# LouisNUST/pose-unsupervised

Hardware: AMD Instinct MI355X
Metric: 4-view 256x256 frames/sec (fwd+triangulate) (higher is better)
Workload: dtype bf16

## Files before the change

pose-unsupervised_amd/csrc/bottleneck.hip:

```cpp
#include "gemm_common.h"

namespace posu {
namespace {

struct BottleGeom {
  const void* x;
  void* y;
  const void* w1;
  const float* s1;
  const float* b1;
  const void* w2;
  const float* s2;
  const float* b2;
  const void* w3;
  const float* s3;
  const float* b3;
  int N, H;
  int strips;
  int rows;
};

#ifndef POSU_BNECK_ABLATE
#define POSU_BNECK_ABLATE 0
#endif
constexpr int kAbl = POSU_BNECK_ABLATE;


constexpr int kP = 64, kW = 64, kC = 256;
constexpr int kW2 = 0;
constexpr int kW3 = 73728;
constexpr int kT1 = 106496;
constexpr int kSlot = 66 * 128;
constexpr int kBN = kT1 + 3 * kSlot;
constexpr int kXP = kBN + 3072;
constexpr int kXT = kXP + 16384;
constexpr int kLds = kXT + 8192;
static_assert(kLds <= 160 * 1024, "LDS");

__device__ __forceinline__ void raw_barrier() {
  if (kAbl & 8) return;
  lds_barrier();
}

__device__ __forceinline__ void ld8(const float* p, float* v) {
  const float4 a = *reinterpret_cast<const float4*>(p);
  const float4 b = *reinterpret_cast<const float4*>(p + 4);
  v[0] = a.x; v[1] = a.y; v[2] = a.z; v[3] = a.w;
  v[4] = b.x; v[5] = b.y; v[6] = b.z; v[7] = b.w;
}

template <typename T, bool DOWN>
__global__ __launch_bounds__(512, 1) void bottleneck64_kernel(BottleGeom g) {
  using O = Op<T>;
  constexpr int ES = static_cast<int>(sizeof(T));
  static_assert(ES == 2, "bf16 / f16 activations");
  constexpr int kCi = DOWN ? 64 : kC;
  constexpr int NF = DOWN ? 2 : 4;
  constexpr int kW3K = DOWN ? 2 * kP : kP;
  __shared__ __attribute__((aligned(16))) char smem[kLds];

  const int tid = threadIdx.x;
  const int lane = tid & 63, wid = tid >> 6;
  const int r16 = lane & 15, q = lane >> 4;
  const int pg = wid & 3, h = wid >> 2;
  const unsigned lds0 = static_cast<unsigned>(reinterpret_cast<size_t>((__attribute__((address_space(3))) char*)smem));
  const unsigned wid_u = __builtin_amdgcn_readfirstlane(static_cast<unsigned>(wid));

  const int n = blockIdx.x / g.strips;
  const int ya = (blockIdx.x - n * g.strips) * g.rows, yb = ya + g.rows;
  const int H = g.H;
  const int px = 16 * pg + r16;
  const int cq = 16 * (q & 1) + 8 * (q >> 1);
  const float* bn = reinterpret_cast<const float*>(smem + kBN);
  float* xp_mine = reinterpret_cast<float*>(smem + kXP + (2 * pg + h) * 2048 + lane * 32);
  const float* xp_part = reinterpret_cast<const float*>(smem + kXP + (2 * pg + 1 - h) * 2048 + lane * 32);
  uint4* xt_mine = reinterpret_cast<uint4*>(smem + kXT + (2 * pg + h) * 1024 + lane * 16);
  const uint4* xt_part = reinterpret_cast<const uint4*>(smem + kXT + (2 * pg + 1 - h) * 1024 + lane * 16);

  {
    const u32x4 w2s = make_srd(g.w2, kP * 9 * kP * ES);
    const u32x4 w3s = make_srd(g.w3, kC * kW3K * ES);
    const int cL = (tid & 7) ^ ((tid >> 4) & 7), drow = tid >> 3;
#pragma unroll
    for (int t = 0; t < 9; ++t)
      dma16(w2s, (drow * (9 * kP) + t * kP + cL * 8) * ES, lds0 + kW2 + t * 8192 + wid_u * 1024);
#pragma unroll
    for (int i = 0; i < 4; ++i)
      dma16(w3s, ((drow + 64 * i) * kW3K + cL * 8) * ES, lds0 + kW3 + i * 8192 + wid_u * 1024);
    float* bw = reinterpret_cast<float*>(smem + kBN);
    if (tid < 64) {
      bw[tid] = g.s1[tid];
      bw[64 + tid] = g.b1[tid];
      bw[128 + tid] = g.s2[tid];
      bw[192 + tid] = g.b2[tid];
    }
    if (tid < 256) {
      bw[256 + tid] = DOWN ? 1.f : g.s3[tid];
      bw[512 + tid] = g.b3[tid];
    }
    if (tid < 48) {
      const int sl = tid >> 4, side = (tid >> 3) & 1, ch = tid & 7;
      *reinterpret_cast<uint4*>(smem + kT1 + sl * kSlot + side * 65 * 128 + ch * 16) = make_uint4(0, 0, 0, 0);
    }
  }
  uint4 w1f[4][4];
  {
    const T* w1 = reinterpret_cast<const T*>(g.w1);
#pragma unroll
    for (int s = 0; s < 4; ++s)
#pragma unroll
      for (int j = 0; j < 4; ++j) {
        if constexpr (DOWN) {
          if (s < 2 && j < 2) w1f[s][j] = *reinterpret_cast<const uint4*>(w1 + (16 * (2 * h + j) + r16) * kCi + 32 * s + 8 * q);
        } else {
          w1f[s][j] = *reinterpret_cast<const uint4*>(w1 + (16 * ((j + 2 * h) & 3) + r16) * kC + 32 * (4 * h + s) + 8 * q);
        }
      }
  }
  uint4 wdf[2][2][4];
  if constexpr (DOWN) {
    const T* w3 = reinterpret_cast<const T*>(g.w3);
#pragma unroll
    for (int qh = 0; qh < 2; ++qh)
#pragma unroll
      for (int s = 0; s < 2; ++s)
#pragma unroll
        for (int j = 0; j < 4; ++j)
          wdf[qh][s][j] = *reinterpret_cast<const uint4*>(w3 + (128 * h + 64 * qh + 16 * j + r16) * kW3K + kP + 32 * s + 8 * q);
  }

  const __amdgpu_buffer_rsrc_t xrs =
      __builtin_amdgcn_make_buffer_rsrc(const_cast<void*>(g.x), 0, g.N * H * kW * kCi * ES, 0x00020000);
  const __amdgpu_buffer_rsrc_t yrs = __builtin_amdgcn_make_buffer_rsrc(g.y, 0, g.N * H * kW * kC * ES, 0x00020000);
  const int lane_off = (px * kC + 128 * h + cq) * ES;
  const int lane_offx = DOWN ? (px * kCi + 8 * q) * ES : lane_off;
  constexpr int kRowBytes = kW * kC * ES, kRowBytesX = kW * kCi * ES;
  const int rmax = (yb < H - 1 ? yb : H - 1);
  auto load_row = [&](int r, uint4(&f)[4]) {
    const int rr = r < 0 ? 0 : (r > rmax ? rmax : r);
    const int roff = __builtin_amdgcn_readfirstlane((n * H + rr) * kRowBytesX);
    if (kAbl & 32) {
#pragma unroll
      for (int s = 0; s < NF; ++s) f[s] = make_uint4(rr, s, lane, 1);
      return;
    }
#pragma unroll
    for (int s = 0; s < NF; ++s) {
      const auto v = __builtin_amdgcn_raw_buffer_load_b128(xrs, lane_offx + 64 * s, roff, (kAbl & 128) ? 2 : 0);
      f[s] = make_uint4(v[0], v[1], v[2], v[3]);
    }
  };
  auto conv1_part = [&](int r, const uint4(&f)[4], f32x4(&acc)[2]) {
    f32x4 a[4];
#pragma unroll
    for (int j = 0; j < 4; ++j) a[j] = f32x4{0.f, 0.f, 0.f, 0.f};
    if constexpr (DOWN) {
      if (r >= 0 && r < H) {
#pragma unroll
        for (int s = 0; s < 2; ++s)
#pragma unroll
          for (int j = 0; j < 2; ++j) O::mma(a[j], w1f[s][j], f[s]);
      }
      acc[0] = a[0];
      acc[1] = a[1];
      return;
    }
    if (r >= 0 && r < H) {
#pragma unroll
      for (int s = 0; s < 4; ++s)
#pragma unroll
        for (int j = 0; j < 4; ++j) {
          if (kAbl & 16) a[j][0] += __uint_as_float(f[s].x ^ w1f[s][j].y);
          else O::mma(a[j], w1f[s][j], f[s]);
        }
    }
    *reinterpret_cast<f32x4*>(xp_mine) = a[2];
    *reinterpret_cast<f32x4*>(xp_mine + 4) = a[3];
    acc[0] = a[0];
    acc[1] = a[1];
  };
  auto conv1_fin = [&](int r, const f32x4(&acc)[2]) {
    char* slot = smem + kT1 + ((r + 3) % 3) * kSlot;
    const bool ok = r >= 0 && r < H;
    f32x4 t0 = acc[0], t1 = acc[1];
    if constexpr (!DOWN) {
      const f32x4 pa = *reinterpret_cast<const f32x4*>(xp_part);
      const f32x4 pb = *reinterpret_cast<const f32x4*>(xp_part + 4);
#pragma unroll
      for (int e = 0; e < 4; ++e) {
        t0[e] += pa[e];
        t1[e] += pb[e];
      }
    }
    const int c0 = 16 * (2 * h + (q & 1)) + 8 * (q >> 1);
    float v[8], sc[8], sh[8];
#pragma unroll
    for (int e = 0; e < 4; ++e) {
      const auto sw = __builtin_amdgcn_permlane16_swap(__float_as_uint(t0[e]), __float_as_uint(t1[e]), false, false);
      v[e] = __uint_as_float(sw[0]);
      v[4 + e] = __uint_as_float(sw[1]);
    }
    ld8(bn + c0, sc);
    ld8(bn + 64 + c0, sh);
    affine8<!DOWN>(v, sc, sh);
#pragma unroll
    for (int e = 0; e < 8; ++e) v[e] = ok ? fmaxf(v[e], 0.f) : 0.f;
    *reinterpret_cast<uint4*>(slot + swz(px + 1, c0 >> 3)) = O::store_vals(v);
  };
  auto conv2_row = [&](int y, auto&& mid) -> uint4 {
    f32x4 acc2[2];
#pragma unroll
    for (int j = 0; j < 2; ++j) acc2[j] = f32x4{0.f, 0.f, 0.f, 0.f};
#pragma unroll
    for (int t = 0; t < 9; ++t) {
      if (t == 5) mid();
      const int dy = t / 3, dx = t % 3;
      const char* slot = smem + kT1 + ((y - 1 + dy + 3) % 3) * kSlot;
      const char* Wt = smem + kW2 + t * 8192;
#pragma unroll
      for (int cb = 0; cb < 2; ++cb) {
        uint4 wf[2];
#pragma unroll
        for (int j = 0; j < 2; ++j) wf[j] = *reinterpret_cast<const uint4*>(Wt + swz(16 * (2 * h + j) + r16, 4 * cb + q));
        const uint4 tf = *reinterpret_cast<const uint4*>(slot + swz(px + dx, 4 * cb + q));
#pragma unroll
        for (int j = 0; j < 2; ++j) {
          if (kAbl & 1) acc2[j][0] += __uint_as_float(wf[j].x ^ tf.y);
          else O::mma(acc2[j], wf[j], tf);
        }
      }
    }
    const int ca = 32 * h + 4 * q, cb2 = ca + 16;
    const float4 sa = *reinterpret_cast<const float4*>(bn + 128 + ca);
    const float4 sb = *reinterpret_cast<const float4*>(bn + 128 + cb2);
    const float4 ha = *reinterpret_cast<const float4*>(bn + 192 + ca);
    const float4 hb = *reinterpret_cast<const float4*>(bn + 192 + cb2);
    const float s8[8] = {sa.x, sa.y, sa.z, sa.w, sb.x, sb.y, sb.z, sb.w};
    const float h8[8] = {ha.x, ha.y, ha.z, ha.w, hb.x, hb.y, hb.z, hb.w};
    float v[8] = {acc2[0][0], acc2[0][1], acc2[0][2], acc2[0][3], acc2[1][0], acc2[1][1], acc2[1][2], acc2[1][3]};
    affine8<!DOWN>(v, s8, h8);
#pragma unroll
    for (int e = 0; e < 8; ++e) v[e] = fmaxf(v[e], 0.f);
    return O::store_vals(v);
  };
  uint4 pend[4];
  int pend_off = 0;
  auto flush = [&](int k) {
    const uint4 u = pend[k];
    if (kAbl & 4) {
      asm volatile("" ::"v"(u.x), "v"(u.y), "v"(u.z), "v"(u.w));
      return;
    }
    __builtin_amdgcn_raw_buffer_store_b128((__attribute__((ext_vector_type(4))) unsigned){u.x, u.y, u.z, u.w}, yrs,
                                           lane_off + 64 * k + pend_off, 0, (kAbl & 64) ? 2 : 0);
  };
  auto conv3_row = [&](int y, const uint4(&tb)[2], const uint4(&res)[4]) {
    pend_off = __builtin_amdgcn_readfirstlane((n * H + y) * kRowBytes);
#pragma unroll
    for (int qh = 0; qh < 2; ++qh) {
      const int qd = 2 * h + qh;
      f32x4 acc3[4];
#pragma unroll
      for (int j = 0; j < 4; ++j) acc3[j] = f32x4{0.f, 0.f, 0.f, 0.f};
#pragma unroll
      for (int kb = 0; kb < 2; ++kb) {
#pragma unroll
        for (int j = 0; j < 4; ++j) {
          const uint4 wf = *reinterpret_cast<const uint4*>(smem + kW3 + swz(64 * qd + 16 * j + r16, 4 * kb + q));
          if (kAbl & 2) acc3[j][0] += __uint_as_float(wf.x ^ tb[kb].y);
          else O::mma(acc3[j], wf, tb[kb]);
        }
      }
      if constexpr (DOWN) {
#pragma unroll
        for (int s = 0; s < 2; ++s)
#pragma unroll
          for (int j = 0; j < 4; ++j) O::mma(acc3[j], wdf[qh][s][j], res[s]);
      }
#pragma unroll
      for (int jp = 0; jp < 2; ++jp) {
        const int s = 2 * qd + jp, c0 = 32 * s + cq;
        float v[8], r[8], sc[8], sh[8];
#pragma unroll
        for (int e = 0; e < 4; ++e) {
          const auto sw = __builtin_amdgcn_permlane16_swap(__float_as_uint(acc3[2 * jp][e]),
                                                           __float_as_uint(acc3[2 * jp + 1][e]), false, false);
          v[e] = __uint_as_float(sw[0]);
          v[4 + e] = __uint_as_float(sw[1]);
        }
        ld8(bn + 512 + c0, sh);
        if constexpr (DOWN) {
#pragma unroll
          for (int e = 0; e < 8; ++e) v[e] = fmaxf(v[e] + sh[e], 0.f);
        } else {
          ld8(bn + 256 + c0, sc);
          O::load_vals(res[2 * qh + jp], r);
          affine8<!DOWN>(v, sc, sh);
          add8<!DOWN>(v, r);
#pragma unroll
          for (int e = 0; e < 8; ++e) v[e] = fmaxf(v[e], 0.f);
        }
        uint4& pk = pend[2 * qh + jp];
        pk = O::store_vals(v);
        asm("" : "+v"(pk.x), "+v"(pk.y), "+v"(pk.z), "+v"(pk.w));
      }
    }
  };

  uint4 xa[4], xb[4], xc[4], xd[4];
  f32x4 c1[2];
  load_row(ya - 1, xd);
  load_row(ya, xa);
  vm_wait<0>();
  raw_barrier();
  load_row(ya + 1, xb);
  load_row(ya + 2, xc);
  conv1_part(ya - 1, xd, c1);
  if (!DOWN) raw_barrier();
  conv1_fin(ya - 1, c1);
  if (!DOWN) raw_barrier();
  conv1_part(ya, xa, c1);
  if (!DOWN) raw_barrier();
  conv1_fin(ya, c1);

  auto step = [&](int y, const uint4(&ra)[4], const uint4(&rb)[4], uint4(&rd)[4], bool fl) {
    conv1_part(y + 1, rb, c1);
    load_row(y + 3, rd);
    if (fl) flush(0);
    if (!DOWN) raw_barrier();
    conv1_fin(y + 1, c1);
    if (fl) flush(1);
    raw_barrier();
    const uint4 mine = conv2_row(y, [&] { if (fl) flush(2); });
    if (fl) flush(3);
    *xt_mine = mine;
    raw_barrier();
    const uint4 part = *xt_part;
    const uint4 tb[2] = {h ? part : mine, h ? mine : part};
    conv3_row(y, tb, ra);
  };
  step(ya, xa, xb, xd, false);
  int y = ya + 1;
  for (; y + 4 <= yb; y += 4) {
    step(y, xb, xc, xa, true);
    step(y + 1, xc, xd, xb, true);
    step(y + 2, xd, xa, xc, true);
    step(y + 3, xa, xb, xd, true);
  }
  if (y < yb) {
    step(y, xb, xc, xa, true);
    if (y + 1 < yb) step(y + 1, xc, xd, xb, true);
    if (y + 2 < yb) step(y + 2, xd, xa, xc, true);
  }
#pragma unroll
  for (int k = 0; k < 4; ++k) flush(k);
}

}
}

using namespace posu;

namespace {
int bottleneck_launch(bool down, int dtype, const void* x, int N, int H, int W, int C, int P, const void* w1,
                      const float* s1, const float* b1, const void* w2, const float* s2, const float* b2,
                      const void* w3, const float* s3, const float* b3, void* y, void* stream, const char* what) {
  const std::string wh(what);
  POSU_REQUIRE(dtype == POSU_BF16 || dtype == POSU_F16, wh + ": dtype must be BF16 or F16");
  POSU_REQUIRE(x && w1 && s1 && b1 && w2 && s2 && b2 && w3 && (s3 || down) && b3 && y, wh + ": null pointer");
  POSU_REQUIRE(x != y, wh + ": the output must not alias the input");
  POSU_REQUIRE(W == kW && C == (down ? 64 : kC) && P == kP,
               wh + (down ? ": built for W = 64, C = 64, planes = 64 (layer1 block 0 of PoseResNet at 256x256)"
                          : ": built for W = 64, C = 256, planes = 64 (layer1 of PoseResNet at 256x256)"));
  POSU_REQUIRE(N > 0 && H > 0, wh + ": empty input");
  POSU_REQUIRE(static_cast<long long>(N) * H * W * kC * 2 < (1LL << 31) - 256,
               wh + ": activation exceeds the 2 GiB addressing range");
  for (const void* p : {x, static_cast<const void*>(y), w1, w2, w3})
    POSU_REQUIRE((reinterpret_cast<size_t>(p) & 15) == 0, wh + ": pointers must be 16-byte aligned");
  BottleGeom g{};
  g.x = x;
  g.y = y;
  g.w1 = w1;
  g.s1 = s1;
  g.b1 = b1;
  g.w2 = w2;
  g.s2 = s2;
  g.b2 = b2;
  g.w3 = w3;
  g.s3 = s3;
  g.b3 = b3;
  g.N = N;
  g.H = H;
  int strips = 1;
  while (N * strips * 2 <= 256 && H % (strips * 2) == 0 && H / (strips * 2) >= 2) strips *= 2;
  g.strips = strips;
  g.rows = H / strips;
  hipStream_t s = as_stream(stream);
  const dim3 grid(N * strips), block(512);
  if (dtype == POSU_BF16) {
    if (down) hipLaunchKernelGGL((bottleneck64_kernel<uint16_t, true>), grid, block, 0, s, g);
    else hipLaunchKernelGGL((bottleneck64_kernel<uint16_t, false>), grid, block, 0, s, g);
  } else {
    if (down) hipLaunchKernelGGL((bottleneck64_kernel<f16_t, true>), grid, block, 0, s, g);
    else hipLaunchKernelGGL((bottleneck64_kernel<f16_t, false>), grid, block, 0, s, g);
  }
  return check_launch(what);
}
}

extern "C" int posu_bottleneck_fwd(int dtype, const void* x, int N, int H, int W, int C, int P, const void* w1,
                                   const float* s1, const float* b1, const void* w2, const float* s2, const float* b2,
                                   const void* w3, const float* s3, const float* b3, void* y, void* stream) {
  return bottleneck_launch(false, dtype, x, N, H, W, C, P, w1, s1, b1, w2, s2, b2, w3, s3, b3, y, stream,
                           "posu_bottleneck_fwd");
}

extern "C" int posu_bottleneck_down_fwd(int dtype, const void* x, int N, int H, int W, int C, int P,
                                        const void* w1, const float* s1, const float* b1, const void* w2,
                                        const float* s2, const float* b2, const void* w3d, const float* shift3,
                                        void* y, void* stream) {
  return bottleneck_launch(true, dtype, x, N, H, W, C, P, w1, s1, b1, w2, s2, b2, w3d, nullptr, shift3, y, stream,
                           "posu_bottleneck_down_fwd");
}
```

Measured before the change: 55700.

## Stagger the two wave teams by one barrier interval in the bottleneck kernel

Remaps the eight waves into two teams and, for the non-downsampling bottleneck, offsets one team by one barrier phase. Team 1 waits an extra barrier at start and team 0 waits one at the end, so the teams run different pipeline stages at once instead of all doing MFMA or all doing memory work together. To allow the lag, conv1 runs two rows ahead, the t1 ring grows from 3 to 4 slots, and the conv2 exchange buffer now shares the conv1 partial-sum scratch area to stay within LDS. The lag depends on slot-reuse timing across barriers, so it risks races and adds extra prologue barriers.

```diff
diff --git a/pose-unsupervised_amd/csrc/bottleneck.hip b/pose-unsupervised_amd/csrc/bottleneck.hip
--- a/pose-unsupervised_amd/csrc/bottleneck.hip
+++ b/pose-unsupervised_amd/csrc/bottleneck.hip
@@ -25,16 +25,27 @@
 #endif
 constexpr int kAbl = POSU_BNECK_ABLATE;
 
+#ifndef POSU_BNECK_STAGGER
+#define POSU_BNECK_STAGGER 1
+#endif
+#ifndef POSU_BNECK_STAGGER_DOWN
+#define POSU_BNECK_STAGGER_DOWN 0
+#endif
+#ifndef POSU_BNECK_TEAMS_DOWN
+#define POSU_BNECK_TEAMS_DOWN 0
+#endif
+#ifndef POSU_BNECK_PRIO
+#define POSU_BNECK_PRIO 0
+#endif
 
 constexpr int kP = 64, kW = 64, kC = 256;
 constexpr int kW2 = 0;
 constexpr int kW3 = 73728;
 constexpr int kT1 = 106496;
 constexpr int kSlot = 66 * 128;
-constexpr int kBN = kT1 + 3 * kSlot;
+constexpr int kBN = kT1 + 4 * kSlot;
 constexpr int kXP = kBN + 3072;
-constexpr int kXT = kXP + 16384;
-constexpr int kLds = kXT + 8192;
+constexpr int kLds = kXP + 16384;
 static_assert(kLds <= 160 * 1024, "LDS");
 
 __device__ __forceinline__ void raw_barrier() {
@@ -57,12 +68,19 @@
   constexpr int kCi = DOWN ? 64 : kC;
   constexpr int NF = DOWN ? 2 : 4;
   constexpr int kW3K = DOWN ? 2 * kP : kP;
+  constexpr int kLag = DOWN ? POSU_BNECK_STAGGER_DOWN : POSU_BNECK_STAGGER;
+  static_assert(kLag == 0 || kLag == 1, "a lag of 2 intervals reuses a ring slot under its last reader (see step)");
+  constexpr bool kTeams = !DOWN || POSU_BNECK_TEAMS_DOWN;
+  static_assert(kTeams || kLag == 0, "the lag needs the two-team wave mapping");
+  constexpr int kAhead = kLag ? 2 : 1;
+  constexpr int kRing = kAhead + 2;
   __shared__ __attribute__((aligned(16))) char smem[kLds];
 
   const int tid = threadIdx.x;
   const int lane = tid & 63, wid = tid >> 6;
   const int r16 = lane & 15, q = lane >> 4;
-  const int pg = wid & 3, h = wid >> 2;
+  const int team = __builtin_amdgcn_readfirstlane(wid >> 2);
+  const int pg = kTeams ? wid >> 1 : wid & 3, h = kTeams ? wid & 1 : wid >> 2;
   const unsigned lds0 = static_cast<unsigned>(reinterpret_cast<size_t>((__attribute__((address_space(3))) char*)smem));
   const unsigned wid_u = __builtin_amdgcn_readfirstlane(static_cast<unsigned>(wid));
 
@@ -72,10 +90,11 @@
   const int px = 16 * pg + r16;
   const int cq = 16 * (q & 1) + 8 * (q >> 1);
   const float* bn = reinterpret_cast<const float*>(smem + kBN);
-  float* xp_mine = reinterpret_cast<float*>(smem + kXP + (2 * pg + h) * 2048 + lane * 32);
-  const float* xp_part = reinterpret_cast<const float*>(smem + kXP + (2 * pg + 1 - h) * 2048 + lane * 32);
-  uint4* xt_mine = reinterpret_cast<uint4*>(smem + kXT + (2 * pg + h) * 1024 + lane * 16);
-  const uint4* xt_part = reinterpret_cast<const uint4*>(smem + kXT + (2 * pg + 1 - h) * 1024 + lane * 16);
+  const int wm = 2 * pg + h, wp = 2 * pg + 1 - h;
+  float* xp_mine = reinterpret_cast<float*>(smem + kXP + wm * 2048 + lane * 32);
+  const float* xp_part = reinterpret_cast<const float*>(smem + kXP + wp * 2048 + lane * 32);
+  uint4* xt_mine = reinterpret_cast<uint4*>(smem + kXP + wp * 2048 + lane * 16);
+  const uint4* xt_part = reinterpret_cast<const uint4*>(smem + kXP + wm * 2048 + lane * 16);
 
   {
     const u32x4 w2s = make_srd(g.w2, kP * 9 * kP * ES);
@@ -98,7 +117,7 @@
       bw[256 + tid] = DOWN ? 1.f : g.s3[tid];
       bw[512 + tid] = g.b3[tid];
     }
-    if (tid < 48) {
+    if (tid < 64) {
       const int sl = tid >> 4, side = (tid >> 3) & 1, ch = tid & 7;
       *reinterpret_cast<uint4*>(smem + kT1 + sl * kSlot + side * 65 * 128 + ch * 16) = make_uint4(0, 0, 0, 0);
     }
@@ -154,8 +173,9 @@
     f32x4 a[4];
 #pragma unroll
     for (int j = 0; j < 4; ++j) a[j] = f32x4{0.f, 0.f, 0.f, 0.f};
+    const bool live = r >= 0 && r < H && r <= yb;
     if constexpr (DOWN) {
-      if (r >= 0 && r < H) {
+      if (live) {
 #pragma unroll
         for (int s = 0; s < 2; ++s)
 #pragma unroll
@@ -165,7 +185,7 @@
       acc[1] = a[1];
       return;
     }
-    if (r >= 0 && r < H) {
+    if (live) {
 #pragma unroll
       for (int s = 0; s < 4; ++s)
 #pragma unroll
@@ -180,7 +200,7 @@
     acc[1] = a[1];
   };
   auto conv1_fin = [&](int r, const f32x4(&acc)[2]) {
-    char* slot = smem + kT1 + ((r + 3) % 3) * kSlot;
+    char* slot = smem + kT1 + ((r + kRing) % kRing) * kSlot;
     const bool ok = r >= 0 && r < H;
     f32x4 t0 = acc[0], t1 = acc[1];
     if constexpr (!DOWN) {
@@ -215,7 +235,7 @@
     for (int t = 0; t < 9; ++t) {
       if (t == 5) mid();
       const int dy = t / 3, dx = t % 3;
-      const char* slot = smem + kT1 + ((y - 1 + dy + 3) % 3) * kSlot;
+      const char* slot = smem + kT1 + ((y - 1 + dy + kRing) % kRing) * kSlot;
       const char* Wt = smem + kW2 + t * 8192;
 #pragma unroll
       for (int cb = 0; cb < 2; ++cb) {
@@ -309,26 +329,39 @@
 
   uint4 xa[4], xb[4], xc[4], xd[4];
   f32x4 c1[2];
+  constexpr bool kBarA = !DOWN || kAhead == 2;
   load_row(ya - 1, xd);
   load_row(ya, xa);
   vm_wait<0>();
   raw_barrier();
   load_row(ya + 1, xb);
   load_row(ya + 2, xc);
+  if (team == 1) {
+    if (POSU_BNECK_PRIO && kLag) __builtin_amdgcn_s_setprio(1);
+#pragma unroll
+    for (int i = 0; i < kLag; ++i) raw_barrier();
+  }
   conv1_part(ya - 1, xd, c1);
-  if (!DOWN) raw_barrier();
+  if (kBarA) raw_barrier();
   conv1_fin(ya - 1, c1);
-  if (!DOWN) raw_barrier();
+  if (kBarA) raw_barrier();
   conv1_part(ya, xa, c1);
-  if (!DOWN) raw_barrier();
+  if (kBarA) raw_barrier();
   conv1_fin(ya, c1);
-
-  auto step = [&](int y, const uint4(&ra)[4], const uint4(&rb)[4], uint4(&rd)[4], bool fl) {
-    conv1_part(y + 1, rb, c1);
+  if (kBarA) raw_barrier();
+  if (kAhead == 2) {
+    conv1_part(ya + 1, xb, c1);
+    if (kBarA) raw_barrier();
+    conv1_fin(ya + 1, c1);
+    if (kBarA) raw_barrier();
+  }
+
+  auto step = [&](int y, const uint4(&ra)[4], const uint4(&rb)[4], const uint4(&rc)[4], uint4(&rd)[4], bool fl) {
+    conv1_part(y + kAhead, kAhead == 2 ? rc : rb, c1);
     load_row(y + 3, rd);
     if (fl) flush(0);
-    if (!DOWN) raw_barrier();
-    conv1_fin(y + 1, c1);
+    if (kBarA) raw_barrier();
+    conv1_fin(y + kAhead, c1);
     if (fl) flush(1);
     raw_barrier();
     const uint4 mine = conv2_row(y, [&] { if (fl) flush(2); });
@@ -336,24 +369,29 @@
     *xt_mine = mine;
     raw_barrier();
     const uint4 part = *xt_part;
+    asm volatile("" ::: "memory");
     const uint4 tb[2] = {h ? part : mine, h ? mine : part};
     conv3_row(y, tb, ra);
   };
-  step(ya, xa, xb, xd, false);
+  step(ya, xa, xb, xc, xd, false);
   int y = ya + 1;
   for (; y + 4 <= yb; y += 4) {
-    step(y, xb, xc, xa, true);
-    step(y + 1, xc, xd, xb, true);
-    step(y + 2, xd, xa, xc, true);
-    step(y + 3, xa, xb, xd, true);
+    step(y, xb, xc, xd, xa, true);
+    step(y + 1, xc, xd, xa, xb, true);
+    step(y + 2, xd, xa, xb, xc, true);
+    step(y + 3, xa, xb, xc, xd, true);
   }
   if (y < yb) {
-    step(y, xb, xc, xa, true);
-    if (y + 1 < yb) step(y + 1, xc, xd, xb, true);
-    if (y + 2 < yb) step(y + 2, xd, xa, xc, true);
+    step(y, xb, xc, xd, xa, true);
+    if (y + 1 < yb) step(y + 1, xc, xd, xa, xb, true);
+    if (y + 2 < yb) step(y + 2, xd, xa, xb, xc, true);
   }
 #pragma unroll
   for (int k = 0; k < 4; ++k) flush(k);
+  if (team == 0) {
+#pragma unroll
+    for (int i = 0; i < kLag; ++i) raw_barrier();
+  }
 }
 
 }
```

New measurement: 55980, median of 6. No clear change (+0.5%).
